# ZpokenWeb3/zk-light-client-implementation

Measured on AMD Instinct MI355X. Metric: Block_i BFT-finality proofs/sec (100 validators), higher is better.
Workload: dtype u64

## Files before the change

zk-light-client-implementation_amd/csrc/plonky2_gates.cuh:

```cuda
#pragma once
#include "gl_ext.cuh"
#include "poseidon_gl.cuh"
#if defined(__HIP_DEVICE_COMPILE__) && !defined(ZKLC_GL_NO_MUL_ASM)
#include "goldilocks_mul_asm.inc"
#endif

#define P2_MAX_CH 2
#define P2_UNUSED_SELECTOR 0xFFFFFFFFULL

enum p2_gate_type {
    P2_NOOP = 0, P2_CONSTANT, P2_PUBLIC_INPUT, P2_ARITHMETIC, P2_ARITHMETIC_EXT, P2_MUL_EXT, P2_BASE_SUM, P2_POSEIDON,
    P2_POSEIDON_MDS, P2_RANDOM_ACCESS, P2_REDUCING, P2_REDUCING_EXT, P2_EXPONENTIATION, P2_COSET_INTERPOLATION,
    P2_U32_ARITHMETIC, P2_U32_ADD_MANY, P2_U32_SUBTRACTION, P2_U32_RANGE_CHECK, P2_COMPARISON,
    P2_U32_INTERLEAVE, P2_UNINTERLEAVE_TO_U32, P2_UNINTERLEAVE_TO_B32, P2_NUM_GATE_TYPES,
    P2_POSEIDON_LAZY = 100,
    P2_POSEIDON_LOOSE = 110
};

struct p2_gate {
    u32 type;
    u32 p[4];
    u32 selector_index, group_start, group_end;
    u32 extra_off;
};
// ... 785 lines not shown
        p2_load<16>(v, 5 * num_ops + 16 * i, l);
        u64 x = r[0], y = r[1], bin = r[2], res = r[3], bout = r[4];
        u64 initial = gl_sub(gl_sub(x, y), bin);
        out.emit(gl_sub(res, gl_add(initial, gl_mul(bout, 1ULL << 32))));
        u64 comb = 0;
        u64 rev[16], rp[16];
#pragma unroll
        for (int j = 0; j < 16; j++) rev[j] = l[15 - j];
        p2_range_products4<16>(rev, rp);
#pragma unroll
        for (int j = 15; j >= 0; j--) {
            out.emit(rp[15 - j]);
            comb = p2_horner4(comb, l[j]);
        }
        out.emit(gl_sub(gl_canonical(comb), res));
        out.emit(gl_mul(bout, gl_sub(1, bout)));
    }
}

template <class V>
ZKLC_D void p2_eval_u32_range_check(const V &v, u32 n, p2_consumer &out) {
    for (u32 i = 0; i < n; i++) {
        u64 l[16];
        p2_load<16>(v, n + 16 * i, l);
        u64 sum = 0;
#pragma unroll
        for (int j = 15; j >= 0; j--) sum = p2_horner4(sum, l[j]);
        out.emit(gl_sub(gl_canonical(sum), v.w(i)));
        u64 rp[16];
        p2_range_products4<16>(l, rp);
#pragma unroll
        for (int j = 0; j < 16; j++) out.emit(rp[j]);
    }
}

template <class V>
ZKLC_D void p2_eval_comparison(const V &v, u32 num_bits, u32 num_chunks, p2_consumer &out) {
    const u32 chunk_bits = (num_bits + num_chunks - 1) / num_chunks;
    const u32 chunk_size = 1u << chunk_bits;
    u64 c1 = 0, c2 = 0;
    {
        u32 i = num_chunks;
        for (; i >= 8; i -= 8) {
            u64 a[8], b[8];
            p2_load<8>(v, 4 + i - 8, a);
            p2_load<8>(v, 4 + num_chunks + i - 8, b);
#pragma unroll
            for (int q = 7; q >= 0; q--) {
                c1 = chunk_size == 4 ? p2_horner4(c1, a[q]) : gl_add(gl_mul(c1, chunk_size), a[q]);
                c2 = chunk_size == 4 ? p2_horner4(c2, b[q]) : gl_add(gl_mul(c2, chunk_size), b[q]);
            }
        }
        while (i-- > 0) {
            c1 = chunk_size == 4 ? p2_horner4(c1, v.w(4 + i)) : gl_add(gl_mul(c1, chunk_size), v.w(4 + i));
            c2 = chunk_size == 4 ? p2_horner4(c2, v.w(4 + num_chunks + i)) : gl_add(gl_mul(c2, chunk_size), v.w(4 + num_chunks + i));
        }
        if (chunk_size == 4) {
            c1 = gl_canonical(c1);
            c2 = gl_canonical(c2);
        }
    }
    out.emit(gl_sub(c1, v.w(0)));
    out.emit(gl_sub(c2, v.w(1)));
    u64 msd = 0;
    auto chunk = [&](u64 a, u64 b, u64 dummy, u64 eq, u64 inter) {
        out.emit(p2_range_product(a, chunk_size));
// ... 105 lines not shown
```

zk-light-client-implementation_amd/csrc/plonky2_prover.hip:

```cpp
#include <algorithm>
#include <chrono>
#include <stdio.h>
#include <stdlib.h>
#include <new>
#include <vector>
#include <string.h>
#include "plonky2_gates.cuh"
#include "plonky2_host.h"
#include "zklc_internal.h"

#define P2_THREADS 256

struct p2_challenges {
    u64 beta[P2_MAX_CH], gamma[P2_MAX_CH], alpha[P2_MAX_CH];
};

__global__ void p2_pow_table_kernel(u64 *out, u64 base, u64 n) {
    u64 i = (u64)blockIdx.x * blockDim.x + threadIdx.x;
    if (i < n) out[i] = gl_pow(base, i);
}

__global__ void p2_scale_by_powers_kernel(u64 *data, u64 base, u64 n) {
    u64 j = (u64)blockIdx.x * blockDim.x + threadIdx.x;
    if (j >= n) return;
    u64 *p = data + (size_t)blockIdx.y * n + j;
    *p = gl_mul(*p, gl_pow(base, j));
}

__global__ void p2_ext_powers_kernel(gl2 *out, gl2 z, u64 n) {
    u64 j = (u64)blockIdx.x * blockDim.x + threadIdx.x;
    if (j < n) out[j] = gl2_pow(z, j);
}

// ... 77 lines not shown
    u32 s = threadIdx.x * per, e = s + per < nblocks ? s + per : nblocks;
    u64 acc = 1;
    for (u32 i = s; i < e; i++) acc = gl_mul(acc, totals[i]);
    sh[threadIdx.x] = acc;
    __syncthreads();
    for (u32 off = 1; off < P2_THREADS; off <<= 1) {
        u64 t = threadIdx.x >= off ? sh[threadIdx.x - off] : 1;
        __syncthreads();
        sh[threadIdx.x] = gl_mul(sh[threadIdx.x], t);
        __syncthreads();
    }
    u64 pre = threadIdx.x ? sh[threadIdx.x - 1] : 1;
    for (u32 i = s; i < e; i++) {
        u64 t = totals[i];
        totals[i] = pre;
        pre = gl_mul(pre, t);
    }
    if (threadIdx.x == P2_THREADS - 1) *grand_total = sh[P2_THREADS - 1];
}
__global__ void __launch_bounds__(P2_THREADS)
p2_z_apply_kernel(const u64 *__restrict__ excl, const u64 *__restrict__ totals, const u64 *__restrict__ rp, u32 n, u32 npp,
                  u64 *__restrict__ z_out, u64 *__restrict__ pp_out) {
    u32 i = blockIdx.x * blockDim.x + threadIdx.x;
    if (i >= n) return;
    u64 z = gl_mul(excl[i], totals[i / P2_SCAN_BLOCK]);
    z_out[i] = z;
    for (u32 k = 0; k < npp; k++) pp_out[(size_t)k * n + i] = gl_mul(z, rp[(size_t)k * n + i]);
}

struct p2_quotient_args {
    const u64 *cs, *wires, *zs;
    const p2_gate *gates;
    const u64 *extra, *k_is;
    u32 lde_bits, degree_bits, rate_bits, num_constants, nsel, routed, nch, npp, qdf, num_gates;
    u64 w_lde;
    u64 zh_inv[16], zh[16];
    u64 n_field;
    u64 pih[4];
    p2_challenges ch;
    const u32 *apow[P2_MAX_CH];
    u64 *out;
    const u64 *xs, *l0;
    u32 num_wires;
};

__global__ void __launch_bounds__(P2_THREADS) p2_quotient_base_kernel(p2_quotient_args a) {
    const size_t N = (size_t)1 << a.lde_bits;
    size_t p = (size_t)blockIdx.x * blockDim.x + threadIdx.x;
    if (p >= N) return;
    u64 i = __brevll((u64)p) >> (64 - a.lde_bits);
    u64 x = a.xs[p];
    const u32 coset = (u32)i & ((1u << a.rate_bits) - 1);
    u64 l0 = a.l0[p];
    u64 i_next = (i + (1ULL << a.rate_bits)) & (N - 1);
    size_t p_next = (size_t)(__brevll(i_next) >> (64 - a.lde_bits));

    p2_consumer out;
    out.nch = a.nch;
    for (int c = 0; c < P2_MAX_CH; c++) out.apow[c] = (gl_ktab *)a.apow[c];
    out.reset(0);
    for (u32 c = 0; c < a.nch; c++) out.emit(gl_mul(l0, gl_sub(a.zs[(size_t)c * N + p], 1)));
    const u32 nchunks = a.npp + 1;
    for (u32 c = 0; c < a.nch; c++) {
        u64 beta = a.ch.beta[c], gamma = a.ch.gamma[c];
        u64 prev = a.zs[(size_t)c * N + p];
        for (u32 k = 0; k < nchunks; k++) {
            u64 np = 1, dp = 1;
            u32 end = (k + 1) * a.qdf < a.routed ? (k + 1) * a.qdf : a.routed;
            gl_ktab64 *kis = (gl_ktab64 *)a.k_is;
            u32 j = k * a.qdf;
            if (end - j == 8) {
                u64 wv[8], sv[8];
#pragma unroll
                for (int q = 0; q < 8; q++) {
                    wv[q] = a.wires[(size_t)(j + q) * N + p];
                    sv[q] = a.cs[(size_t)(a.num_constants + j + q) * N + p];
                }
#pragma unroll
                for (int q = 0; q < 8; q++) {
                    u64 w = gl_add(wv[q], gamma);
                    np = gl_mul(np, gl_add(w, gl_mul(beta, gl_mul(kis[j + q], x))));
                    dp = gl_mul(dp, gl_add(w, gl_mul(beta, sv[q])));
                }
                j = end;
            }
            for (; j < end; j++) {
                u64 w = gl_add(a.wires[(size_t)j * N + p], gamma);
                np = gl_mul(np, gl_add(w, gl_mul(beta, gl_mul(kis[j], x))));
                dp = gl_mul(dp, gl_add(w, gl_mul(beta, a.cs[(size_t)(a.num_constants + j) * N + p])));
            }
            u64 next = k + 1 < nchunks ? a.zs[(size_t)(a.nch + c * a.npp + k) * N + p] : a.zs[(size_t)c * N + p_next];
            out.emit(gl_sub(gl_mul(prev, np), gl_mul(next, dp)));
            prev = next;
        }
    }
    const u64 zi = a.zh_inv[coset];
#pragma unroll
    for (int c = 0; c < P2_MAX_CH; c++)
        if (c < (int)a.nch) a.out[(size_t)c * N + p] = gl_mul(out.result(c), zi);
}

#define P2_GATE_LIST_MAX 8
struct p2_gate_list {
    u32 n, idx[P2_GATE_LIST_MAX];
};
template <int TYPE>
__global__ void __launch_bounds__(P2_THREADS) p2_quotient_gate_kernel(p2_quotient_args a, p2_gate_list list) {
    const size_t N = (size_t)1 << a.lde_bits;
    size_t p = (size_t)blockIdx.x * blockDim.x + threadIdx.x;
    if (p >= N) return;
    u64 i = __brevll((u64)p) >> (64 - a.lde_bits);
    const u32 coset = (u32)i & ((1u << a.rate_bits) - 1);
    p2_vars v;
    v.wires = a.wires;
    v.consts = a.cs;
    v.stride = N;
    v.p = p;
    v.nsel = a.nsel;
    for (int k = 0; k < 4; k++) v.pih[k] = a.pih[k];
    p2_consumer out;
    out.nch = a.nch;
// ... 285 lines not shown
                u64 t = sum[c];
                for (u32 w = 1; w < P2_AMT_WAVES; w++) t = gl_add(t, part[((size_t)w * P2_MAX_CH + c) * 64 + lane]);
                u64 *o = a.out + (size_t)c * N + p;
                *o = gl_add(*o, gl_mul(t, zi));
            }
    }
}
static bool p2_amt_make_plan(const p2_gate *gates, const p2_gate_list &list, p2_amt_plan &plan) {
    if (list.n < 2 || list.n > 2 * P2_AMT_WAVES) return false;
    u32 load[P2_AMT_WAVES] = {0, 0, 0, 0}, used[P2_AMT_WAVES] = {0, 0, 0, 0};
    for (int w = 0; w < P2_AMT_WAVES; w++) plan.slot[w][0] = plan.slot[w][1] = 0xFFFFFFFFu;
    plan.lo = 0xFFFFFFFFu;
    plan.hi = 0;
    bool taken[P2_GATE_LIST_MAX] = {};
    for (u32 r = 0; r < list.n; r++) {
        u32 best = 0xFFFFFFFFu;
        for (u32 t = 0; t < list.n; t++)
            if (!taken[t] && (best == 0xFFFFFFFFu || gates[list.idx[t]].p[1] > gates[list.idx[best]].p[1])) best = t;
        taken[best] = true;
        const p2_gate &g = gates[list.idx[best]];
        const u32 ops = g.p[1], l0 = (g.p[0] + 3) * ops;
        if (ops == 0 || 24 * ops >= 480) return false;
        u32 w = 0xFFFFFFFFu;
        for (u32 k = 0; k < P2_AMT_WAVES; k++)
            if (used[k] < 2 && (w == 0xFFFFFFFFu || load[k] < load[w])) w = k;
        plan.slot[w][used[w]++] = best;
        load[w] += ops;
        plan.lo = l0 < plan.lo ? l0 : plan.lo;
        plan.hi = l0 + 18 * ops > plan.hi ? l0 + 18 * ops : plan.hi;
    }
    return plan.hi > plan.lo;
}

typedef void (*p2_gate_kernel_fn)(p2_quotient_args, p2_gate_list);
static p2_gate_kernel_fn p2_gate_kernel_of(u32 type) {
    static const char *pg = getenv("ZKLC_P2_POSEIDON_GATE");
    if (type == P2_POSEIDON && (!pg || !pg[0] || !strcmp(pg, "loose"))) return p2_quotient_gate_kernel<P2_POSEIDON_LOOSE>;
    if (type == P2_POSEIDON && pg && !strncmp(pg, "lazy", 4)) {
        return pg[4] == '1' ? p2_quotient_gate_kernel<P2_POSEIDON_LAZY + 1> : p2_quotient_gate_kernel<P2_POSEIDON_LAZY>;
    }
    switch (type) {
#define P2_CASE(T) case T: return p2_quotient_gate_kernel<T>;
        P2_CASE(P2_CONSTANT) P2_CASE(P2_PUBLIC_INPUT) P2_CASE(P2_ARITHMETIC) P2_CASE(P2_ARITHMETIC_EXT) P2_CASE(P2_MUL_EXT)
        P2_CASE(P2_BASE_SUM) P2_CASE(P2_POSEIDON) P2_CASE(P2_POSEIDON_MDS) P2_CASE(P2_RANDOM_ACCESS) P2_CASE(P2_REDUCING)
        P2_CASE(P2_REDUCING_EXT) P2_CASE(P2_EXPONENTIATION) P2_CASE(P2_COSET_INTERPOLATION) P2_CASE(P2_U32_ARITHMETIC)
        P2_CASE(P2_U32_ADD_MANY) P2_CASE(P2_U32_SUBTRACTION) P2_CASE(P2_U32_RANGE_CHECK) P2_CASE(P2_COMPARISON)
        P2_CASE(P2_U32_INTERLEAVE) P2_CASE(P2_UNINTERLEAVE_TO_U32) P2_CASE(P2_UNINTERLEAVE_TO_B32)
#undef P2_CASE
        default: return nullptr;
    }
}

#define P2_FQ_MAX_WAVES 8
#define P2_FQ_MAX_JOBS 40
#define P2_JOB_BASE 0xFFFFu
struct p2_fused_plan {
    u32 nwaves;
    u32 njobs[P2_FQ_MAX_WAVES];
    uint16_t jobs[P2_FQ_MAX_WAVES][P2_FQ_MAX_JOBS];
};

__global__ void __launch_bounds__(64 * P2_FQ_MAX_WAVES) p2_quotient_fused_kernel(p2_quotient_args a, p2_fused_plan plan) {
    extern __shared__ u64 p2_tile[];
    const size_t N = (size_t)1 << a.lde_bits;
    const u32 lane = threadIdx.x & 63;
    const u32 wave = __builtin_amdgcn_readfirstlane(threadIdx.x >> 6);
// ... 17 lines not shown
            p2_tile[(size_t)j * 64 + lane] = src[p];
        }
    }
    __syncthreads();
    p2_vars_lds v;
    v.consts = (p2_lds_u64 *)p2_tile;
    v.wires = v.consts + (size_t)a.num_constants * 64;
    v.lane = lane;
    v.nsel = a.nsel;
    for (int k = 0; k < 4; k++) v.pih[k] = a.pih[k];
    u64 sum[P2_MAX_CH] = {0, 0};
    p2_consumer out;
    out.nch = a.nch;
    for (int c = 0; c < P2_MAX_CH; c++) out.apow[c] = (gl_ktab *)a.apow[c];
    const u32 njobs = plan.njobs[wave];
    for (u32 jb = 0; jb < njobs; jb++) {
        const u32 g = plan.jobs[wave][jb];
        if (g == P2_JOB_BASE) {
            u64 i = __brevll((u64)p) >> (64 - a.lde_bits);
            u64 x = a.xs[p], l0 = a.l0[p];
            u64 i_next = (i + (1ULL << a.rate_bits)) & (N - 1);
            size_t p_next = (size_t)(__brevll(i_next) >> (64 - a.lde_bits));
            out.reset(0);
            for (u32 c = 0; c < a.nch; c++) out.emit(gl_mul(l0, gl_sub(a.zs[(size_t)c * N + p], 1)));
            const u32 nchunks = a.npp + 1;
            for (u32 c = 0; c < a.nch; c++) {
                u64 beta = a.ch.beta[c], gamma = a.ch.gamma[c];
                u64 prev = a.zs[(size_t)c * N + p];
                for (u32 k = 0; k < nchunks; k++) {
                    u64 np = 1, dp = 1;
                    u32 end = (k + 1) * a.qdf < a.routed ? (k + 1) * a.qdf : a.routed;
                    for (u32 j = k * a.qdf; j < end; j++) {
                        u64 w = gl_add(v.w(j), gamma);
                        np = gl_mul(np, gl_add(w, gl_mul(beta, gl_mul(a.k_is[j], x))));
                        dp = gl_mul(dp, gl_add(w, gl_mul(beta, a.cs[(size_t)(a.num_constants + j) * N + p])));
                    }
                    u64 next = k + 1 < nchunks ? a.zs[(size_t)(a.nch + c * a.npp + k) * N + p] : a.zs[(size_t)c * N + p_next];
                    out.emit(gl_sub(gl_mul(prev, np), gl_mul(next, dp)));
                    prev = next;
                }
            }
            for (u32 c = 0; c < a.nch; c++) sum[c] = gl_add(sum[c], out.result((int)c));
            continue;
        }
        p2_gate gate = a.gates[g];
        out.reset(a.nch + a.nch * (a.npp + 1));
        p2_eval_gate(gate, v, a.extra, out);
        u64 f = p2_filter(g, gate.group_start, gate.group_end, v.sel(gate.selector_index), a.nsel > 1);
        for (u32 c = 0; c < a.nch; c++) sum[c] = gl_add(sum[c], gl_mul(f, out.result((int)c)));
    }
    u64 *part = p2_tile + (size_t)ncols * 64;
    for (u32 c = 0; c < a.nch; c++) part[((size_t)wave * P2_MAX_CH + c) * 64 + lane] = sum[c];
    __syncthreads();
    if (wave == 0) {
        u64 i = __brevll((u64)p) >> (64 - a.lde_bits);
        const u32 coset = (u32)i & ((1u << a.rate_bits) - 1);
        for (u32 c = 0; c < a.nch; c++) {
            u64 t = sum[c];
            for (u32 w = 1; w < plan.nwaves; w++) t = gl_add(t, part[((size_t)w * P2_MAX_CH + c) * 64 + lane]);
            a.out[(size_t)c * N + p] = gl_mul(t, a.zh_inv[coset]);
        }
    }
}

__global__ void __launch_bounds__(256) p2_point_tables_kernel(u64 *xs, u64 *l0, u32 lde_bits, u32 rate_bits, u64 w_lde, u64 n_field,
                                                               p2_quotient_args zhsrc) {
    const size_t N = (size_t)1 << lde_bits;
// ... 207 lines not shown
        e >>= 1;
    }
    return r;
}
static u64 h_inv(u64 a) { return h_pow(a, GL_P - 2); }
static u64 h_root(u32 log_n) { return h_pow(GL_POWER_OF_TWO_GENERATOR, 1ULL << (32 - log_n)); }
static gl2 h2_mul(gl2 x, gl2 y) {
    return gl2_make(h_add(h_mul(x.a, y.a), h_mul(7, h_mul(x.b, y.b))), h_add(h_mul(x.a, y.b), h_mul(x.b, y.a)));
}
static gl2 h2_add(gl2 x, gl2 y) { return gl2_make(h_add(x.a, y.a), h_add(x.b, y.b)); }
static gl2 h2_pow(gl2 x, u64 e) {
    gl2 r = gl2_make(1, 0);
    while (e) {
        if (e & 1) r = h2_mul(r, x);
        x = h2_mul(x, x);
        e >>= 1;
    }
    return r;
}

struct p2_batch {
    u32 width = 0;
    u64 *coeffs = nullptr, *lde = nullptr, *tree = nullptr;
};

struct zklc_plonky2_circuit {
    zklc_ctx *ctx = nullptr;
    int device = 0;
    zklc_plonky2_params P;
    u32 n = 0, N = 0, lde_bits = 0, nchunks = 0;
    std::vector<p2_gate> gates;
    p2_gate *d_gates = nullptr;
    u64 *d_extra = nullptr, *d_kis = nullptr, *d_subgroup = nullptr, *d_sigma_vals = nullptr;
    p2_batch cs, wires, zs, quot;
    u64 *d_wire_vals = nullptr;
    u64 *d_rp = nullptr, *d_excl = nullptr, *d_totals = nullptr, *d_grand = nullptr;
    u64 *d_qv = nullptr;
    u32 *d_apow = nullptr;
    u32 *d_fri_apow = nullptr;
    u64 *d_xs = nullptr, *d_l0 = nullptr;
    p2_fused_plan plan = {};
    size_t fused_lds = 0;
    std::vector<double> gate_ms;
    gl2 *d_zpow = nullptr, *d_open = nullptr, *d_open_partial = nullptr;
    gl2 *d_fri[9] = {};
    u64 *d_fri_tree[8] = {};
    gl2 *d_final = nullptr;
    unsigned long long *d_found = nullptr;
    p2_gather *d_gather = nullptr;
    u64 *d_gather_out = nullptr;
    size_t gather_cap = 0, gather_out_words = 0;
    std::vector<uint8_t> cap_bytes;
    uint8_t digest[32];
    std::vector<u64> last_challenges;
    double timings[8] = {};
    u64 tree_words = 0;
    std::vector<void *> allocs;
    std::vector<std::pair<uint8_t *, size_t>> pin_blocks;
    size_t pin_used = 0;
};

static bool p2_pin_enabled() {
    static const bool on = !(getenv("ZKLC_PINNED_STAGING") && getenv("ZKLC_PINNED_STAGING")[0] == '0');
    return on;
}
static void p2_pin_free(void *q) {
// ... 132 lines not shown
    a.num_gates = P.num_gates;
    a.num_wires = P.num_wires;
    a.w_lde = h_root(c->lde_bits);
    u64 gn = h_pow(GL_GENERATOR, c->n), w_r = h_root(P.rate_bits);
    for (u32 k = 0; k < (1u << P.rate_bits); k++) {
        a.zh[k] = h_sub(h_mul(gn, h_pow(w_r, k)), 1);
        a.zh_inv[k] = h_inv(a.zh[k]);
    }
    a.n_field = c->n;
    a.xs = c->d_xs;
    a.l0 = c->d_l0;
    a.out = c->d_qv;
}

static int32_t p2_plan_quotient(zklc_plonky2_circuit *c, hipStream_t st) {
    zklc_ctx *ctx = c->ctx;
    const zklc_plonky2_params &P = c->P;
    const u32 N = c->N;
    c->plan.nwaves = 0;
    const char *mode = getenv("ZKLC_P2_QUOTIENT");
    if (!mode || strcmp(mode, "fused")) return ZKLC_OK;
    const size_t tile = (size_t)(P.num_constants + P.num_wires) * 64 * 8;
    if (N < 64 || P.num_gates + 1 > P2_FQ_MAX_WAVES * P2_FQ_MAX_JOBS) return ZKLC_OK;
    u32 nw = tile * 2 + 2 * 4 * P2_MAX_CH * 512 <= 160 * 1024 ? 4 : 8;
    if (const char *e = getenv("ZKLC_P2_FQ_WAVES")) nw = (u32)atoi(e);
    if (nw < 1 || nw > P2_FQ_MAX_WAVES) return ZKLC_ERR_INVALID_ARG;
    c->fused_lds = tile + (size_t)nw * P2_MAX_CH * 64 * 8;
    if (c->fused_lds > 160 * 1024) return ZKLC_OK;
    ZKLC_HIP(ctx, hipFuncSetAttribute((const void *)p2_quotient_fused_kernel, hipFuncAttributeMaxDynamicSharedMemorySize,
                                      (int)c->fused_lds));
    p2_quotient_args a = {};
    p2_quotient_static_args(c, a);
    for (u32 k = 0; k < P2_MAX_CH; k++) a.apow[k] = c->d_apow;
    hipEvent_t e0, e1;
    ZKLC_HIP(ctx, hipEventCreate(&e0));
    ZKLC_HIP(ctx, hipEventCreate(&e1));
    c->gate_ms.assign(P.num_gates + 1, 0.0);
    for (u32 g = 0; g <= P.num_gates; g++) {
        p2_gate_kernel_fn fn = g < P.num_gates ? p2_gate_kernel_of(c->gates[g].type) : nullptr;
        if (g < P.num_gates && !fn) continue;
        for (int rep = 0; rep < 2; rep++) {
            ZKLC_HIP(ctx, hipEventRecord(e0, st));
            if (fn) {
                p2_gate_list one = {};
                one.n = 1;
                one.idx[0] = g;
                hipLaunchKernelGGL(fn, dim3((N + P2_THREADS - 1) / P2_THREADS), dim3(P2_THREADS), 0, st, a, one);
            } else
                hipLaunchKernelGGL(p2_quotient_base_kernel, dim3((N + P2_THREADS - 1) / P2_THREADS), dim3(P2_THREADS), 0, st, a);
            ZKLC_HIP(ctx, hipEventRecord(e1, st));
            ZKLC_HIP(ctx, hipEventSynchronize(e1));
            float ms = 0;
            ZKLC_HIP(ctx, hipEventElapsedTime(&ms, e0, e1));
            if (rep == 0 || ms < c->gate_ms[g]) c->gate_ms[g] = ms;
        }
    }
    (void)hipEventDestroy(e0);
    (void)hipEventDestroy(e1);
    std::vector<u32> order;
    for (u32 g = 0; g <= P.num_gates; g++)
        if (g == P.num_gates || p2_gate_kernel_of(c->gates[g].type)) order.push_back(g);
    std::sort(order.begin(), order.end(), [&](u32 x, u32 y) { return c->gate_ms[x] > c->gate_ms[y]; });
    double load[P2_FQ_MAX_WAVES] = {};
    p2_fused_plan plan = {};
    for (u32 g : order) {
        u32 best = 0;
// ... 29 lines not shown
                         zklc_plonky2_circuit *c) {
    const zklc_plonky2_params &P = *params;
    c->ctx = ctx;
    c->device = ctx->device;
    c->P = P;
    c->n = 1u << P.degree_bits;
    c->lde_bits = P.degree_bits + P.rate_bits;
    c->N = 1u << c->lde_bits;
    c->nchunks = P.num_partial_products + 1;
    const u32 n = c->n, N = c->N;
    hipStream_t st = ctx->stream;
    ZKLC_HIP(ctx, hipSetDevice(ctx->device));
    c->gates.resize(P.num_gates);
    for (u32 i = 0; i < P.num_gates; i++) {
        p2_gate g;
        g.type = gates[i].type;
        for (int k = 0; k < 4; k++) g.p[k] = gates[i].p[k];
        g.selector_index = gates[i].selector_index;
        g.group_start = gates[i].group_start;
        g.group_end = gates[i].group_end;
        g.extra_off = gates[i].extra_off;
        if (g.type >= P2_NUM_GATE_TYPES || g.selector_index >= P.num_selectors) return ZKLC_ERR_INVALID_ARG;
        if (g.type == P2_RANDOM_ACCESS && g.p[0] > 6) return ZKLC_ERR_INVALID_ARG;
        if (g.type == P2_COSET_INTERPOLATION && (g.p[0] > 5 || g.p[1] < 2 || g.extra_off + (2u << g.p[0]) > gate_extra_words))
            return ZKLC_ERR_INVALID_ARG;
        c->gates[i] = g;
    }
    P2_ALLOC(c, c->d_gates, sizeof(p2_gate) * P.num_gates);
    ZKLC_HIP(ctx, hipMemcpyAsync(c->d_gates, c->gates.data(), sizeof(p2_gate) * P.num_gates, hipMemcpyHostToDevice, st));
    P2_ALLOC(c, c->d_extra, (size_t)gate_extra_words * 8);
    if (gate_extra_words) ZKLC_HIP(ctx, hipMemcpyAsync(c->d_extra, gate_extra, (size_t)gate_extra_words * 8, hipMemcpyHostToDevice, st));
    P2_ALLOC(c, c->d_kis, (size_t)P.num_routed_wires * 8);
    ZKLC_HIP(ctx, hipMemcpyAsync(c->d_kis, k_is, (size_t)P.num_routed_wires * 8, hipMemcpyHostToDevice, st));
    const u32 nch_ = P.num_challenges;
    P2_ALLOC(c, c->d_subgroup, (size_t)n * 8);
    hipLaunchKernelGGL(p2_pow_table_kernel, dim3((n + 255) / 256), dim3(256), 0, st, c->d_subgroup, h_root(P.degree_bits), (u64)n);
    ZKLC_HIP(ctx, hipGetLastError());

    c->tree_words = zklc_gl_merkle_tree_words(c->lde_bits, P.cap_height < c->lde_bits ? P.cap_height : c->lde_bits);
    auto alloc_batch = [&](p2_batch &b, u32 width) -> int32_t {
        b.width = width;
        P2_ALLOC(c, b.coeffs, (size_t)width * n * 8);
        P2_ALLOC(c, b.lde, (size_t)width * N * 8);
        P2_ALLOC(c, b.tree, c->tree_words * 8);
        return ZKLC_OK;
    };
    const u32 nch = P.num_challenges;
    P2_RC(alloc_batch(c->cs, P.num_constants + P.num_routed_wires));
    P2_RC(alloc_batch(c->wires, P.num_wires));
    P2_RC(alloc_batch(c->zs, nch * (1 + P.num_partial_products)));
    c->quot.width = nch * P.quotient_degree_factor;
    P2_ALLOC(c, c->d_qv, (size_t)nch * N * 8);
    c->quot.coeffs = c->d_qv;
    P2_ALLOC(c, c->quot.lde, (size_t)c->quot.width * N * 8);
    P2_ALLOC(c, c->quot.tree, c->tree_words * 8);
    P2_ALLOC(c, c->d_wire_vals, (size_t)P.num_wires * n * 8);
    P2_ALLOC(c, c->d_sigma_vals, (size_t)P.num_routed_wires * n * 8);
    P2_ALLOC(c, c->d_rp, (size_t)c->nchunks * n * 8);
    P2_ALLOC(c, c->d_excl, (size_t)n * 8);
    P2_ALLOC(c, c->d_totals, (size_t)((n + P2_SCAN_BLOCK - 1) / P2_SCAN_BLOCK) * 8);
    P2_ALLOC(c, c->d_grand, 8);
    P2_ALLOC(c, c->d_apow, (size_t)nch_ * (nch_ + nch_ * (P.num_partial_products + 1) + P.num_gate_constraints + 1) * 24);
    P2_ALLOC(c, c->d_zpow, (size_t)n * sizeof(gl2));
    P2_ALLOC(c, c->d_fri_apow, (size_t)(c->cs.width + c->wires.width + c->zs.width + c->quot.width + 1) * 12 * sizeof(u32));
    P2_ALLOC(c, c->d_xs, (size_t)N * 8);
    P2_ALLOC(c, c->d_l0, (size_t)N * 8);
    u32 total_polys = c->cs.width + c->wires.width + c->zs.width + c->quot.width + nch;
    P2_ALLOC(c, c->d_open, (size_t)total_polys * sizeof(gl2));
    P2_ALLOC(c, c->d_open_partial, (size_t)total_polys * P2_EVAL_SPLIT * sizeof(gl2));
    u32 bits = c->lde_bits;
    P2_ALLOC(c, c->d_fri[0], (size_t)N * sizeof(gl2));
    for (u32 r = 0; r < P.num_arities; r++) {
        u32 leaves_bits = bits - P.arity_bits[r];
        u32 cap_h = P.cap_height < leaves_bits ? P.cap_height : leaves_bits;
        P2_ALLOC(c, c->d_fri_tree[r], zklc_gl_merkle_tree_words(leaves_bits, cap_h) * 8);
        bits = leaves_bits;
        P2_ALLOC(c, c->d_fri[r + 1], ((size_t)1 << bits) * sizeof(gl2));
    }
    P2_ALLOC(c, c->d_final, ((size_t)1 << bits) * sizeof(gl2));
    P2_ALLOC(c, c->d_found, 8);

    size_t cbytes = (size_t)P.num_constants * n * 8, sbytes = (size_t)P.num_routed_wires * n * 8;
    ZKLC_HIP(ctx, hipMemcpyAsync(c->cs.coeffs, constants, cbytes, hipMemcpyHostToDevice, st));
    ZKLC_HIP(ctx, hipMemcpyAsync(c->cs.coeffs + (size_t)P.num_constants * n, sigmas, sbytes, hipMemcpyHostToDevice, st));
    ZKLC_HIP(ctx, hipMemcpyAsync(c->d_sigma_vals, sigmas, sbytes, hipMemcpyHostToDevice, st));
    P2_RC(p2_commit_values(c, st, c->cs, c->cap_bytes));
    {
        p2_quotient_args a = {};
        p2_quotient_static_args(c, a);
        hipLaunchKernelGGL(p2_point_tables_kernel, dim3((N / 4 + 255) / 256 ? (N / 4 + 255) / 256 : 1), dim3(256), 0, st, c->d_xs, c->d_l0,
                           c->lde_bits, P.rate_bits, a.w_lde, a.n_field, a);
        ZKLC_HIP(ctx, hipGetLastError());
        P2_RC(p2_plan_quotient(c, st));
    }

// ... 155 lines not shown
    u32 nblocks = (n + P2_SCAN_BLOCK - 1) / P2_SCAN_BLOCK;
    P2_PIN(c, grand, u64, P2_MAX_CH);
    for (u32 k = 0; k < P2_MAX_CH; k++) grand[k] = 1;
    for (u32 k = 0; k < nch; k++) {
        hipLaunchKernelGGL(p2_chunk_products_kernel, dim3((n + P2_THREADS - 1) / P2_THREADS), dim3(P2_THREADS), 0, st, d_wires,
                           (const u64 *)c->d_sigma_vals, (const u64 *)c->d_subgroup, (const u64 *)c->d_kis, n, P.num_routed_wires,
                           P.quotient_degree_factor, c->nchunks, chal.beta[k], chal.gamma[k], c->d_rp);
        hipLaunchKernelGGL(p2_scan_local_kernel, dim3(nblocks), dim3(P2_THREADS), 0, st, (const u64 *)(c->d_rp + (size_t)npp * n),
                           c->d_excl, c->d_totals, n);
        hipLaunchKernelGGL(p2_scan_totals_kernel, dim3(1), dim3(P2_THREADS), 0, st, c->d_totals, nblocks, c->d_grand);
        hipLaunchKernelGGL(p2_z_apply_kernel, dim3((n + P2_THREADS - 1) / P2_THREADS), dim3(P2_THREADS), 0, st, (const u64 *)c->d_excl,
                           (const u64 *)c->d_totals, (const u64 *)c->d_rp, n, npp, c->zs.coeffs + (size_t)k * n,
                           c->zs.coeffs + (size_t)(nch + k * npp) * n);
        ZKLC_HIP(ctx, hipGetLastError());
        ZKLC_HIP(ctx, zklc_readback_async(&grand[k], c->d_grand, 8, st));
    }
    P2_RC(p2_commit_values(c, st, c->zs, zs_cap));
    for (u32 k = 0; k < nch; k++)
        if (grand[k] != 1) {
            ctx->last_err = "plonky2: the witness violates the copy constraints (permutation product != 1)";
            return ZKLC_ERR_INVALID_ARG;
        }
    p2_observe_cap(ch, zs_cap, hasher);
    for (u32 k = 0; k < nch; k++) chal.alpha[k] = ch.challenge();
    lap(1);

    {
        p2_quotient_args a = {};
        p2_quotient_static_args(c, a);
        for (int k = 0; k < 4; k++) a.pih[k] = pih[k];
        a.ch = chal;
        {
            u32 n_pow = nch + nch * (npp + 1) + P.num_gate_constraints + 1;
            P2_PIN(c, tab, u32, (size_t)nch * n_pow * 6);
            for (u32 k = 0; k < nch; k++) {
                u64 v = 1;
                for (u32 i = 0; i < n_pow; i++) {
                    u32 *t6 = &tab[((size_t)k * n_pow + i) * 6];
                    const u64 v2 = h_mul(v, 1ULL << 32);
                    t6[0] = (u32)(v & 0x3FFFFF), t6[1] = (u32)((v >> 22) & 0x3FFFFF), t6[2] = (u32)(v >> 44);
                    t6[3] = (u32)(v2 & 0x3FFFFF), t6[4] = (u32)((v2 >> 22) & 0x3FFFFF), t6[5] = (u32)(v2 >> 44);
                    v = h_mul(v, chal.alpha[k]);
                }
            }
            ZKLC_HIP(ctx, hipMemcpyAsync(c->d_apow, tab, (size_t)nch * n_pow * 6 * 4, hipMemcpyHostToDevice, st));
            for (u32 k = 0; k < nch; k++) a.apow[k] = c->d_apow + (size_t)k * n_pow * 6;
            for (u32 k = nch; k < P2_MAX_CH; k++) a.apow[k] = c->d_apow;
        }
        if (c->plan.nwaves) {
            hipLaunchKernelGGL(p2_quotient_fused_kernel, dim3(N / 64), dim3(64 * c->plan.nwaves), c->fused_lds, st, a, c->plan);
        } else {
            hipLaunchKernelGGL(p2_quotient_base_kernel, dim3((N + P2_THREADS - 1) / P2_THREADS), dim3(P2_THREADS), 0, st, a);
            static const bool one_per_launch = getenv("ZKLC_P2_GATE_LAUNCH") && !strcmp(getenv("ZKLC_P2_GATE_LAUNCH"), "single");
            std::vector<bool> done(P.num_gates, false);
            for (u32 g = 0; g < P.num_gates; g++) {
                p2_gate_kernel_fn fn = p2_gate_kernel_of(c->gates[g].type);
                if (!fn || done[g]) continue;
                p2_gate_list list = {};
                for (u32 h = g; h < P.num_gates && list.n < (one_per_launch ? 1u : (u32)P2_GATE_LIST_MAX); h++)
                    if (!done[h] && c->gates[h].type == c->gates[g].type) {
                        list.idx[list.n++] = h;
                        done[h] = true;
                    }
                static const bool am_multi = getenv("ZKLC_P2_ADDMANY") && !strcmp(getenv("ZKLC_P2_ADDMANY"), "multi");
                static const bool am_pergate = getenv("ZKLC_P2_ADDMANY") && !strcmp(getenv("ZKLC_P2_ADDMANY"), "pergate");
                static const bool am_check = getenv("ZKLC_P2_ADDMANY") && !strcmp(getenv("ZKLC_P2_ADDMANY"), "check");
                if (am_check && c->gates[g].type == P2_U32_ADD_MANY && N >= 64) {
                    p2_amt_plan plan;
                    if (p2_amt_make_plan(c->gates.data(), list, plan)) {
                        u64 *s1 = nullptr, *s2 = nullptr;
                        const size_t words = (size_t)nch * N;
                        ZKLC_HIP(ctx, hipMalloc(&s1, words * 8));
                        ZKLC_HIP(ctx, hipMalloc(&s2, words * 8));
                        ZKLC_HIP(ctx, hipMemsetAsync(s1, 0, words * 8, st));
                        ZKLC_HIP(ctx, hipMemsetAsync(s2, 0, words * 8, st));
                        p2_quotient_args b1 = a, b2 = a;
                        b1.out = s1;
                        b2.out = s2;
                        hipLaunchKernelGGL(fn, dim3((N + P2_THREADS - 1) / P2_THREADS), dim3(P2_THREADS), 0, st, b1, list);
                        hipLaunchKernelGGL(p2_quotient_addmany_tile_kernel, dim3(N / 64), dim3(64 * P2_AMT_WAVES), 0, st, b2, list, plan);
                        std::vector<u64> h1(words), h2(words);
                        ZKLC_HIP(ctx, hipMemcpyAsync(h1.data(), s1, words * 8, hipMemcpyDeviceToHost, st));
                        ZKLC_HIP(ctx, hipMemcpyAsync(h2.data(), s2, words * 8, hipMemcpyDeviceToHost, st));
                        ZKLC_HIP(ctx, zklc_stream_wait(st));
                        size_t bad = 0;
                        for (size_t i = 0; i < words; i++) bad += h1[i] % GL_P != h2[i] % GL_P;
                        fprintf(stderr, "[zklc] addmany check: %u variants, limb columns [%u, %u): %zu of %zu values differ\n", list.n, plan.lo,
// ... 311 lines not shown
```

Before: 0.2116.

## Add LDS-tiled multi-gate u32 quotient kernel and precompute beta*k_i on host

Adds an opt-in kernel that evaluates several u32 arithmetic, subtraction, range-check and add-many gates together. It stages shared wire columns and their range products in LDS tiles across six waves, prefetching the next tile while the current one is consumed. Separately, it precomputes beta*k_i per challenge on the host and uploads it with the alpha power table, saving one field multiply per routed wire in the permutation terms. The tiled kernel is gated behind an environment variable, and the precompute adds a small host loop and extra transfer.

Result: no change. 0.2125, median of 6 (+0.4%).

```diff
diff --git a/zk-light-client-implementation_amd/csrc/plonky2_gates.cuh b/zk-light-client-implementation_amd/csrc/plonky2_gates.cuh
--- a/zk-light-client-implementation_amd/csrc/plonky2_gates.cuh
+++ b/zk-light-client-implementation_amd/csrc/plonky2_gates.cuh
@@ -841,6 +841,204 @@
 #pragma unroll
         for (int j = 0; j < 16; j++) out.emit(rp[j]);
     }
+}
+
+#define P2_U32T_WAVES 6
+#define P2_U32T_SLOTS 2
+#define P2_U32T_COLS 48u
+struct p2_u32t_cons {
+    u32 gate;
+    u32 type, ops, na;
+    u32 l0, len, split;
+    u32 kper, ktop;
+    int kdir;
+    u32 e_split, e_zero;
+};
+struct p2_u32t_plan {
+    p2_u32t_cons slot[P2_U32T_WAVES][P2_U32T_SLOTS];
+    u32 lo, hi;
+};
+static inline bool p2_u32t_describe(const p2_gate &g, u32 gate_index, p2_u32t_cons &d) {
+    d.gate = gate_index;
+    d.type = g.type;
+    d.na = 0;
+    d.kdir = 1;
+    d.e_split = 0;
+    switch (g.type) {
+        case P2_U32_ADD_MANY:
+            d.na = g.p[0], d.ops = g.p[1], d.l0 = (g.p[0] + 3) * g.p[1], d.len = 18, d.split = 16;
+            d.kper = 21, d.ktop = 1, d.e_split = 20, d.e_zero = 19;
+            return true;
+        case P2_U32_ARITHMETIC:
+            d.ops = g.p[0], d.l0 = 6 * g.p[0], d.len = 32, d.split = 16;
+            d.kper = 36, d.ktop = 2, d.e_split = 35, d.e_zero = 34;
+            return true;
+        case P2_U32_SUBTRACTION:
+            d.ops = g.p[0], d.l0 = 5 * g.p[0], d.len = 16, d.split = 16;
+            d.kper = 19, d.ktop = 1, d.e_zero = 17;
+            return true;
+        case P2_U32_RANGE_CHECK:
+            d.ops = g.p[0], d.l0 = g.p[0], d.len = 16, d.split = 16;
+            d.kper = 17, d.ktop = 16, d.kdir = -1, d.e_zero = 0;
+            return true;
+        default: return false;
+    }
+}
+static inline bool p2_u32t_make_plan(const p2_gate *gates, u32 num_gates, u32 num_wires, bool skip_addmany, p2_u32t_plan &plan, bool *placed) {
+    const u32 MAXC = P2_U32T_WAVES * P2_U32T_SLOTS;
+    p2_u32t_cons best[P2_U32T_WAVES * P2_U32T_SLOTS];
+    u32 nb = 0;
+    for (u32 g = 0; g < num_gates; g++) {
+        placed[g] = false;
+        p2_u32t_cons d;
+        if (!p2_u32t_describe(gates[g], g, d)) continue;
+        if (skip_addmany && d.type == P2_U32_ADD_MANY) continue;
+        if (d.ops == 0 || d.ops > 64 || d.l0 + d.len * d.ops > num_wires || (d.kper + 3) * d.ops >= 480) continue;
+        u32 pos = nb;
+        while (pos > 0 && best[pos - 1].kper * best[pos - 1].ops < d.kper * d.ops) pos--;
+        if (pos >= MAXC) continue;
+        for (u32 t = (nb < MAXC ? nb : MAXC - 1); t > pos; t--) best[t] = best[t - 1];
+        best[pos] = d;
+        if (nb < MAXC) nb++;
+    }
+    if (nb < 2) return false;
+    u32 load[P2_U32T_WAVES], used[P2_U32T_WAVES];
+    for (u32 w = 0; w < P2_U32T_WAVES; w++) {
+        load[w] = used[w] = 0;
+        for (u32 s = 0; s < P2_U32T_SLOTS; s++) {
+            plan.slot[w][s] = p2_u32t_cons();
+            plan.slot[w][s].gate = 0xFFFFFFFFu;
+        }
+    }
+    plan.lo = 0xFFFFFFFFu;
+    plan.hi = 0;
+    for (u32 r = 0; r < nb; r++) {
+        const p2_u32t_cons &d = best[r];
+        u32 w = 0xFFFFFFFFu;
+        for (u32 k = 0; k < P2_U32T_WAVES; k++)
+            if (used[k] < P2_U32T_SLOTS && (w == 0xFFFFFFFFu || load[k] < load[w])) w = k;
+        plan.slot[w][used[w]++] = d;
+        load[w] += d.kper * d.ops;
+        placed[d.gate] = true;
+        plan.lo = d.l0 < plan.lo ? d.l0 : plan.lo;
+        plan.hi = d.l0 + d.len * d.ops > plan.hi ? d.l0 + d.len * d.ops : plan.hi;
+    }
+    return plan.hi > plan.lo;
+}
+template <int S, class V>
+ZKLC_D void p2_u32t_routed(gl_acc3 (&acc)[2][P2_MAX_CH], const V &pv, const p2_u32t_cons &d, gl_ktab *const (&apow)[P2_MAX_CH], int nch, u32 k0) {
+    if (d.type == P2_U32_ADD_MANY) {
+        p2_amt_routed<S>(acc, pv, d.na, d.ops, apow, nch, k0);
+        return;
+    }
+#if defined(__HIPCC__)
+#pragma unroll 1
+#endif
+    for (u32 i = 0; i < d.ops; i++) {
+        u64 e[4];
+        u32 ke[4], ne;
+        if (d.type == P2_U32_ARITHMETIC) {
+            u64 r[6];
+            p2_load<6>(pv, 6 * i, r);
+            const u64 hi_not_max = gl_sub(gl_mul(r[5], gl_sub(0xFFFFFFFFULL, r[4])), 1);
+            e[0] = gl_mul(hi_not_max, r[3]);
+            e[1] = gl_sub(gl_add(gl_mul(r[4], 1ULL << 32), r[3]), gl_add(gl_mul(r[0], r[1]), r[2]));
+            e[2] = gl_neg(r[3]);
+            e[3] = gl_neg(r[4]);
+            ke[0] = 0, ke[1] = 1, ke[2] = 34, ke[3] = 35, ne = 4;
+        } else if (d.type == P2_U32_SUBTRACTION) {
+            u64 r[5];
+            p2_load<5>(pv, 5 * i, r);
+            e[0] = gl_sub(r[3], gl_add(gl_sub(gl_sub(r[0], r[1]), r[2]), gl_mul(r[4], 1ULL << 32)));
+            e[1] = gl_neg(r[3]);
+            e[2] = gl_mul(r[4], gl_sub(1, r[4]));
+            e[3] = 0;
+            ke[0] = 0, ke[1] = 17, ke[2] = 18, ke[3] = 18, ne = 3;
+        } else {
+            e[0] = gl_neg(pv.w(i));
+            e[1] = e[2] = e[3] = 0;
+            ke[0] = ke[1] = ke[2] = ke[3] = 0, ne = 1;
+        }
+#pragma unroll
+        for (int t = 0; t < 4; t++)
+            if (t < (int)ne) {
+#pragma unroll
+                for (int c = 0; c < P2_MAX_CH; c++)
+                    if (c < nch) gl_acc3_mul(acc[S][c], e[t], apow[c] + 6 * (size_t)(k0 + d.kper * i + ke[t]));
+            }
+    }
+}
+template <int S>
+ZKLC_D void p2_u32t_consume(gl_acc3 (&acc)[2][P2_MAX_CH], u64 (&comb)[2], const p2_u32t_cons &d, u32 base, u32 top, const u64 *tw,
+                            const u64 *trp, u32 lane, gl_ktab *const (&apow)[P2_MAX_CH], int nch, u32 k0) {
+    const u32 r_end = d.l0 + d.len * d.ops;
+    const u32 c_hi = top < r_end ? top : r_end, c_lo = base > d.l0 ? base : d.l0;
+    if (c_hi <= c_lo) return;
+    const int kdir = d.kdir;
+    const u32 split = d.split, e_split = d.e_split, e_zero = d.e_zero;
+    auto emit = [&](u32 k, u64 val) __attribute__((always_inline)) {
+#pragma unroll
+        for (int c = 0; c < P2_MAX_CH; c++)
+            if (c < nch) gl_acc3_mul(acc[S][c], val, apow[c] + 6 * (size_t)(k0 + k));
+    };
+    u64 cb = comb[S];
+    auto horner = [&](u64 w, u32 kr, u32 lj) __attribute__((always_inline)) {
+        cb = p2_horner4(cb, w);
+        const bool split_done = lj == split, zero_done = lj == 0;
+        if (split_done | zero_done) {
+            emit(kr + (zero_done ? e_zero : e_split), gl_canonical(cb));
+            cb = 0;
+        }
+    };
+    u32 c = c_hi;
+    u32 i = (c - 1 - d.l0) / d.len, l = (c - 1 - d.l0) - d.len * i;
+#if defined(__HIPCC__)
+#pragma unroll 1
+#endif
+    while (c > c_lo) {
+        u32 cnt = l + 1;
+        if (cnt > c - c_lo) cnt = c - c_lo;
+        const u32 kr = d.kper * i;
+        const int kb = (int)(kr + d.ktop) + kdir * (int)(d.len - 1 - l);
+        u32 q = 0;
+#if defined(__HIPCC__)
+#pragma unroll 1
+#endif
+        for (; q + 4 <= cnt; q += 4) {
+            u64 w[4], rp[4];
+#pragma unroll
+            for (int j = 0; j < 4; j++) {
+                const u32 col = c - 1 - q - j - base;
+                w[j] = tw[(size_t)col * 64 + lane];
+                rp[j] = trp[(size_t)col * 64 + lane];
+            }
+#pragma unroll
+            for (int ch = 0; ch < P2_MAX_CH; ch++)
+                if (ch < nch) {
+                    gl_ktab *t = apow[ch] + 6 * (size_t)(k0 + (u32)(kb + kdir * (int)q));
+                    const ptrdiff_t st = 6 * kdir;
+#pragma unroll
+                    for (int j = 0; j < 4; j++) gl_acc3_mul(acc[S][ch], rp[j], t + st * j);
+                }
+#pragma unroll
+            for (int j = 0; j < 4; j++) horner(w[j], kr, l - q - j);
+        }
+#if defined(__HIPCC__)
+#pragma unroll 1
+#endif
+        for (; q < cnt; q++) {
+            const u32 col = c - 1 - q - base;
+            const u64 w = tw[(size_t)col * 64 + lane], rp = trp[(size_t)col * 64 + lane];
+            emit((u32)(kb + kdir * (int)q), rp);
+            horner(w, kr, l - q);
+        }
+        c -= cnt;
+        if (cnt == l + 1) {
+            i--;
+            l = d.len - 1;
+        }
+    }
+    comb[S] = cb;
 }
 
 template <class V>
diff --git a/zk-light-client-implementation_amd/csrc/plonky2_prover.hip b/zk-light-client-implementation_amd/csrc/plonky2_prover.hip
--- a/zk-light-client-implementation_amd/csrc/plonky2_prover.hip
+++ b/zk-light-client-implementation_amd/csrc/plonky2_prover.hip
@@ -1,4 +1,5 @@
 #include <algorithm>
+#include <memory>
 #include <chrono>
 #include <stdio.h>
 #include <stdlib.h>
@@ -142,6 +143,7 @@
     const u64 *cs, *wires, *zs;
     const p2_gate *gates;
     const u64 *extra, *k_is;
+    const u64 *beta_k;
     u32 lde_bits, degree_bits, rate_bits, num_constants, nsel, routed, nch, npp, qdf, num_gates;
     u64 w_lde;
     u64 zh_inv[16], zh[16];
@@ -177,7 +179,7 @@
         for (u32 k = 0; k < nchunks; k++) {
             u64 np = 1, dp = 1;
             u32 end = (k + 1) * a.qdf < a.routed ? (k + 1) * a.qdf : a.routed;
-            gl_ktab64 *kis = (gl_ktab64 *)a.k_is;
+            gl_ktab64 *bk = (gl_ktab64 *)a.beta_k + (size_t)c * a.routed;
             u32 j = k * a.qdf;
             if (end - j == 8) {
                 u64 wv[8], sv[8];
@@ -189,14 +191,14 @@
 #pragma unroll
                 for (int q = 0; q < 8; q++) {
                     u64 w = gl_add(wv[q], gamma);
-                    np = gl_mul(np, gl_add(w, gl_mul(beta, gl_mul(kis[j + q], x))));
+                    np = gl_mul(np, gl_add(w, gl_mul(bk[j + q], x)));
                     dp = gl_mul(dp, gl_add(w, gl_mul(beta, sv[q])));
                 }
                 j = end;
             }
             for (; j < end; j++) {
                 u64 w = gl_add(a.wires[(size_t)j * N + p], gamma);
-                np = gl_mul(np, gl_add(w, gl_mul(beta, gl_mul(kis[j], x))));
+                np = gl_mul(np, gl_add(w, gl_mul(bk[j], x)));
                 dp = gl_mul(dp, gl_add(w, gl_mul(beta, a.cs[(size_t)(a.num_constants + j) * N + p])));
             }
             u64 next = k + 1 < nchunks ? a.zs[(size_t)(a.nch + c * a.npp + k) * N + p] : a.zs[(size_t)c * N + p_next];
@@ -548,6 +550,111 @@
     return plan.hi > plan.lo;
 }
 
+__global__ void __launch_bounds__(64 * P2_U32T_WAVES) p2_quotient_u32_tile_kernel(p2_quotient_args a, p2_u32t_plan plan) {
+    __shared__ u64 tw[P2_U32T_COLS * 64], trp[P2_U32T_COLS * 64];
+    const size_t N = (size_t)1 << a.lde_bits;
+    const u32 lane = threadIdx.x & 63;
+    const u32 wave = __builtin_amdgcn_readfirstlane(threadIdx.x >> 6);
+    const size_t p = (size_t)blockIdx.x * 64 + lane;
+    const u64 *W = a.wires + p;
+    const u32 k0 = a.nch + a.nch * (a.npp + 1);
+    gl_acc3 acc[2][P2_MAX_CH];
+    u64 comb[2] = {0, 0};
+    gl_ktab *apow[P2_MAX_CH];
+#pragma unroll
+    for (int c = 0; c < P2_MAX_CH; c++) apow[c] = (gl_ktab *)a.apow[c];
+    const p2_u32t_cons d0 = plan.slot[wave][0], d1 = plan.slot[wave][1];
+#pragma unroll
+    for (int s = 0; s < 2; s++)
+#pragma unroll
+        for (int c = 0; c < P2_MAX_CH; c++) acc[s][c].c0 = acc[s][c].c1 = acc[s][c].c2 = 0;
+    {
+        p2_vars pv;
+        pv.wires = a.wires;
+        pv.stride = N;
+        pv.p = p;
+        if (d0.gate != 0xFFFFFFFFu) p2_u32t_routed<0>(acc, pv, d0, apow, (int)a.nch, k0);
+        if (d1.gate != 0xFFFFFFFFu) p2_u32t_routed<1>(acc, pv, d1, apow, (int)a.nch, k0);
+    }
+    const u32 per_wave = P2_U32T_COLS / P2_U32T_WAVES;
+    u64 wn[per_wave];
+    u32 top = plan.hi, base = top - plan.lo > P2_U32T_COLS ? top - P2_U32T_COLS : plan.lo;
+#pragma unroll
+    for (u32 j = 0; j < per_wave; j++) {
+        const u32 first = base + wave * per_wave;
+        const u32 col = first + j < top ? first + j : top - 1;
+        wn[j] = W[(size_t)col * N];
+    }
+#pragma unroll 1
+    while (true) {
+        {
+            u64 w[per_wave], rp[per_wave];
+            const u32 first = base + wave * per_wave;
+#pragma unroll
+            for (u32 j = 0; j < per_wave; j++) w[j] = wn[j];
+            p2_range_products4<per_wave>(w, rp);
+#pragma unroll
+            for (u32 j = 0; j < per_wave; j++)
+                if (first + j < top) {
+                    tw[(size_t)(first + j - base) * 64 + lane] = w[j];
+                    trp[(size_t)(first + j - base) * 64 + lane] = rp[j];
+                }
+        }
+        __syncthreads();
+        const u32 ntop = base;
+        const bool more = ntop > plan.lo;
+        const u32 nbase = !more ? plan.lo : (ntop - plan.lo > P2_U32T_COLS ? ntop - P2_U32T_COLS : plan.lo);
+        if (more) {
+            const u32 first = nbase + wave * per_wave;
+#pragma unroll
+            for (u32 j = 0; j < per_wave; j++) {
+                const u32 col = first + j < ntop ? first + j : ntop - 1;
+                wn[j] = W[(size_t)col * N];
+            }
+        }
+        if (d0.gate != 0xFFFFFFFFu) p2_u32t_consume<0>(acc, comb, d0, base, top, tw, trp, lane, apow, (int)a.nch, k0);
+        if (d1.gate != 0xFFFFFFFFu) p2_u32t_consume<1>(acc, comb, d1, base, top, tw, trp, lane, apow, (int)a.nch, k0);
+        __syncthreads();
+        if (!more) break;
+        top = ntop;
+        base = nbase;
+    }
+    u64 sum[P2_MAX_CH];
+#pragma unroll
+    for (int c = 0; c < P2_MAX_CH; c++) sum[c] = 0;
+    p2_vars sv;
+    sv.consts = a.cs;
+    sv.stride = N;
+    sv.p = p;
+    sv.nsel = a.nsel;
+#pragma unroll
+    for (int s = 0; s < 2; s++) {
+        const u32 gi = s == 0 ? d0.gate : d1.gate;
+        if (gi == 0xFFFFFFFFu) continue;
+        const p2_gate g = a.gates[gi];
+        const u64 f = p2_filter(gi, g.group_start, g.group_end, sv.sel(g.selector_index), a.nsel > 1);
+#pragma unroll
+        for (int c = 0; c < P2_MAX_CH; c++)
+            if (c < (int)a.nch) sum[c] = gl_add(sum[c], gl_mul(f, gl_acc3_reduce(acc[s][c])));
+    }
+    u64 *part = tw;
+#pragma unroll
+    for (int c = 0; c < P2_MAX_CH; c++) part[((size_t)wave * P2_MAX_CH + c) * 64 + lane] = sum[c];
+    __syncthreads();
+    if (wave == 0) {
+        const u64 pi = __brevll((u64)p) >> (64 - a.lde_bits);
+        const u64 zi = a.zh_inv[(u32)pi & ((1u << a.rate_bits) - 1)];
+#pragma unroll
+        for (int c = 0; c < P2_MAX_CH; c++)
+            if (c < (int)a.nch) {
+                u64 t = sum[c];
+                for (u32 w = 1; w < P2_U32T_WAVES; w++) t = gl_add(t, part[((size_t)w * P2_MAX_CH + c) * 64 + lane]);
+                u64 *o = a.out + (size_t)c * N + p;
+                *o = gl_add(*o, gl_mul(t, zi));
+            }
+    }
+}
+
 typedef void (*p2_gate_kernel_fn)(p2_quotient_args, p2_gate_list);
 static p2_gate_kernel_fn p2_gate_kernel_of(u32 type) {
     static const char *pg = getenv("ZKLC_P2_POSEIDON_GATE");
@@ -631,7 +738,7 @@
                     u32 end = (k + 1) * a.qdf < a.routed ? (k + 1) * a.qdf : a.routed;
                     for (u32 j = k * a.qdf; j < end; j++) {
                         u64 w = gl_add(v.w(j), gamma);
-                        np = gl_mul(np, gl_add(w, gl_mul(beta, gl_mul(a.k_is[j], x))));
+                        np = gl_mul(np, gl_add(w, gl_mul(a.beta_k[(size_t)c * a.routed + j], x)));
                         dp = gl_mul(dp, gl_add(w, gl_mul(beta, a.cs[(size_t)(a.num_constants + j) * N + p])));
                     }
                     u64 next = k + 1 < nchunks ? a.zs[(size_t)(a.nch + c * a.npp + k) * N + p] : a.zs[(size_t)c * N + p_next];
@@ -905,6 +1012,7 @@
     std::vector<p2_gate> gates;
     p2_gate *d_gates = nullptr;
     u64 *d_extra = nullptr, *d_kis = nullptr, *d_subgroup = nullptr, *d_sigma_vals = nullptr;
+    std::vector<u64> h_kis;
     p2_batch cs, wires, zs, quot;
     u64 *d_wire_vals = nullptr;
     u64 *d_rp = nullptr, *d_excl = nullptr, *d_totals = nullptr, *d_grand = nullptr;
@@ -1103,6 +1211,7 @@
     p2_quotient_args a = {};
     p2_quotient_static_args(c, a);
     for (u32 k = 0; k < P2_MAX_CH; k++) a.apow[k] = c->d_apow;
+    a.beta_k = (const u64 *)c->d_apow;
     hipEvent_t e0, e1;
     ZKLC_HIP(ctx, hipEventCreate(&e0));
     ZKLC_HIP(ctx, hipEventCreate(&e1));
@@ -1198,6 +1307,7 @@
     if (gate_extra_words) ZKLC_HIP(ctx, hipMemcpyAsync(c->d_extra, gate_extra, (size_t)gate_extra_words * 8, hipMemcpyHostToDevice, st));
     P2_ALLOC(c, c->d_kis, (size_t)P.num_routed_wires * 8);
     ZKLC_HIP(ctx, hipMemcpyAsync(c->d_kis, k_is, (size_t)P.num_routed_wires * 8, hipMemcpyHostToDevice, st));
+    c->h_kis.assign(k_is, k_is + P.num_routed_wires);
     const u32 nch_ = P.num_challenges;
     P2_ALLOC(c, c->d_subgroup, (size_t)n * 8);
     hipLaunchKernelGGL(p2_pow_table_kernel, dim3((n + 255) / 256), dim3(256), 0, st, c->d_subgroup, h_root(P.degree_bits), (u64)n);
@@ -1226,7 +1336,8 @@
     P2_ALLOC(c, c->d_excl, (size_t)n * 8);
     P2_ALLOC(c, c->d_totals, (size_t)((n + P2_SCAN_BLOCK - 1) / P2_SCAN_BLOCK) * 8);
     P2_ALLOC(c, c->d_grand, 8);
-    P2_ALLOC(c, c->d_apow, (size_t)nch_ * (nch_ + nch_ * (P.num_partial_products + 1) + P.num_gate_constraints + 1) * 24);
+    P2_ALLOC(c, c->d_apow, (size_t)nch_ * (nch_ + nch_ * (P.num_partial_products + 1) + P.num_gate_constraints + 1) * 24 +
+                               (size_t)nch_ * P.num_routed_wires * 8);
     P2_ALLOC(c, c->d_zpow, (size_t)n * sizeof(gl2));
     P2_ALLOC(c, c->d_fri_apow, (size_t)(c->cs.width + c->wires.width + c->zs.width + c->quot.width + 1) * 12 * sizeof(u32));
     P2_ALLOC(c, c->d_xs, (size_t)N * 8);
@@ -1448,7 +1559,7 @@
         a.ch = chal;
         {
             u32 n_pow = nch + nch * (npp + 1) + P.num_gate_constraints + 1;
-            P2_PIN(c, tab, u32, (size_t)nch * n_pow * 6);
+            P2_PIN(c, tab, u32, (size_t)nch * n_pow * 6 + (size_t)nch * P.num_routed_wires * 2);
             for (u32 k = 0; k < nch; k++) {
                 u64 v = 1;
                 for (u32 i = 0; i < n_pow; i++) {
@@ -1459,7 +1570,11 @@
                     v = h_mul(v, chal.alpha[k]);
                 }
             }
-            ZKLC_HIP(ctx, hipMemcpyAsync(c->d_apow, tab, (size_t)nch * n_pow * 6 * 4, hipMemcpyHostToDevice, st));
+            u64 *bk = (u64 *)(tab + (size_t)nch * n_pow * 6);
+            for (u32 k = 0; k < nch; k++)
+                for (u32 j = 0; j < P.num_routed_wires; j++) bk[(size_t)k * P.num_routed_wires + j] = h_mul(chal.beta[k], c->h_kis[j]);
+            ZKLC_HIP(ctx, hipMemcpyAsync(c->d_apow, tab, (size_t)nch * n_pow * 24 + (size_t)nch * P.num_routed_wires * 8, hipMemcpyHostToDevice, st));
+            a.beta_k = (const u64 *)(c->d_apow + (size_t)nch * n_pow * 6);
             for (u32 k = 0; k < nch; k++) a.apow[k] = c->d_apow + (size_t)k * n_pow * 6;
             for (u32 k = nch; k < P2_MAX_CH; k++) a.apow[k] = c->d_apow;
         }
@@ -1469,6 +1584,16 @@
             hipLaunchKernelGGL(p2_quotient_base_kernel, dim3((N + P2_THREADS - 1) / P2_THREADS), dim3(P2_THREADS), 0, st, a);
             static const bool one_per_launch = getenv("ZKLC_P2_GATE_LAUNCH") && !strcmp(getenv("ZKLC_P2_GATE_LAUNCH"), "single");
             std::vector<bool> done(P.num_gates, false);
+            {
+                static const bool u32t_off = !(getenv("ZKLC_P2_U32TILE") && getenv("ZKLC_P2_U32TILE")[0] == '1');
+                static const bool am_set = getenv("ZKLC_P2_ADDMANY") && getenv("ZKLC_P2_ADDMANY")[0];
+                p2_u32t_plan uplan;
+                std::unique_ptr<bool[]> placed(new bool[P.num_gates]);
+                if (!u32t_off && !one_per_launch && N >= 64 && p2_u32t_make_plan(c->gates.data(), P.num_gates, P.num_wires, am_set, uplan, placed.get())) {
+                    hipLaunchKernelGGL(p2_quotient_u32_tile_kernel, dim3(N / 64), dim3(64 * P2_U32T_WAVES), 0, st, a, uplan);
+                    for (u32 g = 0; g < P.num_gates; g++) done[g] = placed[g];
+                }
+            }
             for (u32 g = 0; g < P.num_gates; g++) {
                 p2_gate_kernel_fn fn = p2_gate_kernel_of(c->gates[g].type);
                 if (!fn || done[g]) continue;
```
